# nktoan/h-edit

Hardware: AMD Instinct MI355X
Metric: edited images/sec (512^2, 50 steps, K Langevin) (higher is better)
Workload: dtype bf16

## Files before the change

h-edit_amd/csrc/store.h:

```cpp
#pragma once
#include <map>
#include <string>
#include <vector>

#include "../../include/hedit.h"
#include "common.h"

#pragma GCC visibility push(hidden)

enum class Pack {
  F32,
  Linear,
  Conv3,
  GegluRows,
  GegluBias,
  FfnLayer,
  FfnBias,
  ChainLayer,
  LinearT,
  Conv3Dgrad,
  Conv3S2Dgrad,
  FlipOIHW,
};

struct PackDst {
  Pack kind;
  void* dst;
  float scale = 1.f;
  long ld = 0;
  int which = 0, lay = 0;
};

struct ParamSlot {
  std::string name;
  size_t numel;
  int O, I;
  int ndim;
  int dims[4];
  bool loaded;
  PackDst to;
  std::vector<PackDst> more;
};

struct ParamStore {
  bool alloc_failed = false;
  bool finalized = false;
  std::vector<void*> owned;
  std::vector<ParamSlot> slots;
  std::map<std::string, int> index;
};

void* store_alloc(ParamStore* h, size_t bytes);
void store_free(ParamStore* h);
template <class T>
T* dalloc(ParamStore* h, size_t n) { return reinterpret_cast<T*>(store_alloc(h, n * sizeof(T))); }

ParamSlot& add_slot(ParamStore* h, const std::string& name, Pack kind, void* dst, size_t numel, int O, int I, int ndim,
                    int d0, int d1, int d2, int d3);
float* vec(ParamStore* h, const std::string& name, int n, float* dst = nullptr);
float* mat(ParamStore* h, const std::string& name, int O, int I);
float* f32conv(ParamStore* h, const std::string& name, int O, int I, int k);
bf16_t* lin(ParamStore* h, const std::string& name, int O, int I, bool conv1x1 = false, bf16_t* dst = nullptr, float scale = 1.f);
bf16_t* conv3(ParamStore* h, const std::string& name, int O, int I);
void* add_dst(ParamStore* h, Pack kind, void* dst, size_t bytes, float scale, long ld);
template <class T>
T* twin(ParamStore* h, Pack kind, size_t n, T* dst = nullptr, float scale = 1.f, long ld = 0) {
  return reinterpret_cast<T*>(add_dst(h, kind, dst, n * sizeof(T), scale, ld));
}

// ... 46 lines not shown
```

h-edit_amd/csrc/store.hip:

```cpp
#include "store.h"

#include "kernels.h"

#define TRY(expr)                        \
  do {                                   \
    int _rc = (expr);                    \
    if (_rc != HEDIT_OK) return _rc;     \
  } while (0)

void* store_alloc(ParamStore* h, size_t bytes) {
  void* p = nullptr;
  if (hipMalloc(&p, bytes > 0 ? bytes : 16) != hipSuccess) {
    h->alloc_failed = true;
    return nullptr;
  }
  h->owned.push_back(p);
  return p;
}

void store_free(ParamStore* h) {
  for (void* p : h->owned) if (p) (void)hipFree(p);
  h->owned.clear();
}

// ... 39 lines not shown

static int pack(const ParamSlot& s, const PackDst& d, const float* w, hipStream_t st) {
  bf16_t* d16 = reinterpret_cast<bf16_t*>(d.dst);
  float* d32 = reinterpret_cast<float*>(d.dst);
  switch (d.kind) {
    case Pack::F32: HIP_TRY(hipMemcpyAsync(d.dst, w, s.numel * sizeof(float), hipMemcpyDeviceToDevice, st)); return HEDIT_OK;
    case Pack::Linear: return pack_linear_launch(w, d16, (long)s.numel, d.scale, st);
    case Pack::Conv3: return pack_conv3x3_launch(w, d16, s.O, s.I, st);
    case Pack::GegluRows: return pack_geglu_rows_launch(w, d16, nullptr, s.O, s.I, st);
    case Pack::GegluBias: return pack_geglu_rows_launch(w, nullptr, d32, (int)s.numel, 1, st);
    case Pack::FfnLayer: return ffn_pack_launch(w, d.which, 1, 1, d16, st);
    case Pack::FfnBias: return ffn_pack_bias_launch(w, d32, st);
    case Pack::ChainLayer: return lin_chain_pack_launch(w, d.which, d.scale, d.lay, d16, st);
    case Pack::LinearT: return pack_linear_t_launch(w, d16, s.O, s.I, st, d.scale, d.ld);
    case Pack::Conv3Dgrad: return pack_conv3x3_dgrad_launch(w, d16, s.O, s.I, st);
    case Pack::Conv3S2Dgrad: return pack_conv3x3_s2_dgrad_launch(w, d16, s.O, s.I, st);
    case Pack::FlipOIHW: return flip_oihw_launch(w, d32, s.O, s.I, s.dims[2], st);
  }
  return HEDIT_ERR_STATE;
}

int store_load(ParamStore* h, const char* what, const char* name, const float* w, size_t numel, hipStream_t st) {
  h->finalized = false;
  auto it = h->index.find(name);
  if (it == h->index.end()) {
    hedit_set_error(std::string("unknown ") + what + (*what ? " " : "") + "parameter: " + name);
    return HEDIT_ERR_ARG;
  }
  ParamSlot& s = h->slots[it->second];
  if (s.numel != numel) {
    hedit_set_error(std::string("size mismatch for ") + name + ": expected " + std::to_string(s.numel) + ", got " + std::to_string(numel));
    return HEDIT_ERR_ARG;
  }
  TRY(pack(s, s.to, w, st));
  for (const PackDst& d : s.more) TRY(pack(s, d, w, st));
  s.loaded = true;
  return HEDIT_OK;
}

int store_missing(const ParamStore* h) {
  int m = 0;
  for (auto& s : h->slots) m += s.loaded ? 0 : 1;
  return m;
}
int store_num_params(const ParamStore* h) { return h ? (int)h->slots.size() : 0; }
const char* store_param_name(const ParamStore* h, int i) {
// ... 33 lines not shown
```

h-edit_amd/csrc/unet.hip:

```cpp
#include <array>
#include <map>
#include <string>
#include <vector>

#include "exec.h"
#include "kernels.h"
#include "store.h"

namespace {

struct Res {
  int cin, cout, temb_off;
  float *n1g, *n1b, *n2g, *n2b, *conv2_b, *sc_b;
  bf16_t *conv1, *conv2, *sc_w;
  bf16_t *conv1_t = nullptr, *conv2_t = nullptr, *sc_t = nullptr;
};

struct Attn {
  int C;
  float *gn_g, *gn_b, *pin_b, *ln1g, *ln1b, *ln2g, *ln2b, *ln3g, *ln3b, *o1_b, *o2_b, *ff1_b, *ff2_b, *pout_b;
  bf16_t *pin, *w_qk, *w_v1, *w_o1, *w_q2, *w_k2, *w_v2, *w_o2, *ff1, *ff2, *pout;
  bf16_t *frs = nullptr, *k1s = nullptr, *ffs = nullptr;
  float* ff1_bp = nullptr;
  int ctx_off = 0;
// ... 14 lines not shown

}

struct HEDIT_HANDLE hedit_unet : ParamStore {
  hedit_unet_cfg cfg;
  int temb_dim = 0, temb_total = 0;
  float *conv_in_w = nullptr, *conv_in_b = nullptr, *te1_b = nullptr, *te2_b = nullptr;
  bf16_t *te1_w = nullptr, *te2_w = nullptr, *temb_w_all = nullptr, *conv_out_w = nullptr;
  float *temb_b_all = nullptr, *conv1_b_all = nullptr, *gn_out_g = nullptr, *gn_out_b = nullptr, *conv_out_b = nullptr;
  std::vector<Block> down, up;
  Res mid_res[2];
  Attn mid_attn;
  int32_t* iota = nullptr;
  int iota_cap = 0;
  bool prof_on = false;
  std::vector<hipEvent_t> prof_pool;
  struct ProfRec { int kind; double flops, bytes; int e0, e1; int m = 0, n = 0, k = 0, tag = 0; };
  std::vector<ProfRec> prof_recs;
  size_t prof_next = 0;
  hedit_attn_hook_fn hook = nullptr;
  void* hook_user = nullptr;
  bf16_t *wk2_all = nullptr, *wv2_all = nullptr;
  int ctx_n = 0, ctx_next = 0;
  std::map<std::array<int, 4>, size_t> ws_cache;
  bool grad = false;
  bf16_t* conv_in_t = nullptr;
  float *conv_out_t = nullptr, *zero_bias = nullptr;
  void* tape = nullptr;
  void (*tape_free)(void*) = nullptr;
  bf16_t* wkv2_t = nullptr;
};

namespace {

void grad_lin(hedit_unet* h, int O, int I, float scale, bf16_t** t, bf16_t** fwd = nullptr) {
  if (!h->grad) return;
  *t = twin<bf16_t>(h, Pack::LinearT, (size_t)O * I, nullptr, scale);
  if (fwd) *fwd = twin<bf16_t>(h, Pack::Linear, (size_t)O * I, *fwd, scale);
}

Res make_res(hedit_unet* h, const std::string& pre, int cin, int cout, int& temb_off) {
  Res r{};
  r.cin = cin; r.cout = cout; r.temb_off = temb_off;
  r.n1g = vec(h, pre + ".norm1.weight", cin);
  r.n1b = vec(h, pre + ".norm1.bias", cin);
  r.conv1 = conv3(h, pre + ".conv1.weight", cout, cin);
// ... 495 lines not shown
}

int broadcast_stem(Fwd& f, size_t row_elems, bf16_t** x, bf16_t** t1, bf16_t** q2, int D) {
  bf16_t** narrow[3] = {x, t1, q2};
  bf16_t* wide[3];
  const void* src[3];
  void* dst[3];
  for (int i = 0; i < 3; ++i) {
    TRY(aalloc(f, &wide[i], (size_t)f.B * row_elems));
    src[i] = *narrow[i];
    dst[i] = wide[i];
  }
  {
    ProfScope ps(f, PK_OTHER, 0.0, 3.0 * (D + f.B) * (double)row_elems * sizeof(bf16_t));
    RUN(f, gather_rows_launch(src, dst, 3, f.B, (long)(row_elems * sizeof(bf16_t)), *f.map, f.st));
  }
  for (int i = 0; i < 3; ++i) {
    f.ar.free(*narrow[i]);
    *narrow[i] = wide[i];
  }
  return HEDIT_OK;
}

int forward_impl(hedit_unet* h, const float* x, float t, const float* ctx, int B, int H0, int W0,
                 const hedit_p2p_plan* plan, float* eps_out, void* ws, size_t ws_bytes, hipStream_t st,
                 bool dry, size_t* peak, int D = 0, const RowMap* map = nullptr) {
  const hedit_unet_cfg& c = h->cfg;
  Fwd f;
  f.h = h; f.B = B; f.st = st; f.plan = plan; f.map = map;
  f.ar.base = reinterpret_cast<char*>(ws); f.ar.cap = ws_bytes; f.ar.dry = dry;
  const int ch0 = c.block_out_channels[0];

  if (!dry && h->iota_cap < B) {
    hedit_set_error("batch larger than " + std::to_string(h->iota_cap) + " rows");
    return HEDIT_ERR_ARG;
  }

  bf16_t* ctxb;
  TRY(aalloc(f, &ctxb, (size_t)B * HEDIT_CTXP * c.cross_attention_dim));
  RUN(f, ctx_pad_launch(ctx, ctxb, B, c.cross_attention_dim, st));
  f.ctxb = ctxb;
  {
    const int MC = B * HEDIT_CTXP;
    bf16_t *k2a, *vt2a;
    TRY(aalloc(f, &k2a, (size_t)MC * h->ctx_n));
    TRY(aalloc(f, &vt2a, (size_t)MC * h->ctx_n));
    TRY(linear(f, ctxb, MC, c.cross_attention_dim, h->wk2_all, h->ctx_n, nullptr, nullptr, k2a, h->ctx_n));
    TRY(linear(f, h->wv2_all, h->ctx_n, c.cross_attention_dim, ctxb, MC, nullptr, nullptr, vt2a, MC, 2));
    f.k2_all = k2a;
    f.vt2_all = vt2a;
  }

  float *te0, *te1, *te2, *temb_all;
  TRY(aalloc(f, &te0, (size_t)ch0));
  TRY(aalloc(f, &te1, (size_t)h->temb_dim));
  TRY(aalloc(f, &te2, (size_t)h->temb_dim));
  TRY(aalloc(f, &temb_all, (size_t)h->temb_total));
  RUN(f, timestep_embed_launch(t, te0, ch0, st));
  RUN(f, gemv_launch(h->te1_w, te0, h->te1_b, nullptr, te1, h->temb_dim, ch0, 0, st));
  RUN(f, gemv_launch(h->te2_w, te1, h->te2_b, nullptr, te2, h->temb_dim, h->temb_dim, 1, st));
  RUN(f, gemv_launch(h->temb_w_all, te2, h->temb_b_all, h->conv1_b_all, temb_all, h->temb_total, h->temb_dim, 1, st));
  f.temb_all = temb_all;

  int H = H0, W = W0;
  const bool share = D > 0 && stem_shareable(h, plan, D, B, H0 * W0);
  float* xrows = nullptr;
  if (D > 0 && !share) {
    const size_t img = (size_t)c.in_channels * H * W;
    TRY(aalloc(f, &xrows, (size_t)B * img));
    const void* src[1] = {x};
    void* dst[1] = {xrows};
    ProfScope ps(f, PK_OTHER, 0.0, (double)(D + B) * img * sizeof(float));
    RUN(f, gather_rows_launch(src, dst, 1, B, (long)(img * sizeof(float)), *map, st));
// ... 123 lines not shown
      const size_t M = (size_t)B * H * W;
      TRY(aalloc(f, &prod, M * 4));
      GemmParams p{};
      p.mode = 1; p.Hin = H; p.Win = W; p.Cin = ch0; p.Hout = H; p.Wout = W;
      p.A = a; p.W = h->conv_out_w; p.M = (int)M; p.N = 4; p.K = 9 * ch0; p.lda = ch0; p.raw_f32 = prod; p.ldc = 4;
      TRY(run_gemm(f, p));
      RUN(f, rows_to_nchw_launch(prod, h->conv_out_b, eps_out, B, (long)H * W, 4, 4, st));
      f.ar.free(prod);
    }
    f.ar.free(a);
    f.ar.free(cur);
  }
  if (peak) *peak = f.ar.peak;
  return HEDIT_OK;
}

}

#include "unetgrad.h"

static void unet_pre_destroy(hedit_unet* h) {
  drop_tape(h);
  for (hipEvent_t e : h->prof_pool) (void)hipEventDestroy(e);
}
HEDIT_LIFECYCLE(unet, hedit_unet, "", unet_pre_destroy)

static int create_impl(const hedit_unet_cfg* cfg, hedit_unet** out, bool grad, bool ctx = false) {
  ARG_CHECK(cfg && out, "null");
  ARG_CHECK(cfg->n_levels >= 2 && cfg->n_levels <= HEDIT_MAX_LEVELS, "n_levels");
  ARG_CHECK(cfg->in_channels <= 8 && cfg->out_channels <= 4, "in/out channels");
  ARG_CHECK(cfg->cross_attention_dim % 64 == 0, "cross_attention_dim % 64");
  for (int i = 0; i < cfg->n_levels; ++i) {
    ARG_CHECK(cfg->block_out_channels[i] % 64 == 0, "block_out_channels % 64");
    ARG_CHECK(cfg->block_out_channels[i] % cfg->norm_num_groups == 0, "channels % groups");
    const int d = cfg->block_out_channels[i] / cfg->heads;
    ARG_CHECK(d == 32 || d == 40 || d == 64 || d == 80 || d == 160, "head dim must be one of 32,40,64,80,160");
  }
  TRY(gemm_prepare());
  if (grad) ARG_CHECK(cfg->in_channels <= 4, "the input-gradient pass needs in_channels <= 4");
  hedit_unet* h = new hedit_unet();
  h->cfg = *cfg;
  h->grad = grad;
  const int* ch = cfg->block_out_channels;
  const int L = cfg->layers_per_block, n = cfg->n_levels;
  h->temb_dim = ch[0] * 4;

// ... 116 lines not shown
  return create_impl(cfg, out, true, true);
} catch (...) { return hedit_abi_catch(); }

int hedit_unet_param_bf16_exact(const hedit_unet* h, int i) try {
  return store_param_bf16_exact(h, i);
} catch (...) { (void)hedit_abi_catch(); return 0; }

size_t hedit_unet_workspace_bytes(hedit_unet* h, int B, int height, int width) try {
  if (!h) return 0;
  const std::array<int, 4> key{B, height, width, h->hook ? 1 : 0};
  auto it = h->ws_cache.find(key);
  if (it != h->ws_cache.end()) return it->second;
  size_t need = 0;
  for (int D = 0; D <= (B <= HEDIT_ROWMAP_MAX ? B : 0); ++D) {
    size_t peak = 0;
    if (forward_impl(h, nullptr, 0.f, nullptr, B, height, width, nullptr, nullptr, nullptr, 0, nullptr, true, &peak, D) != HEDIT_OK) return 0;
    if (peak > need) need = peak;
  }
  need += 4096;
  h->ws_cache[key] = need;
  return need;
} catch (...) { (void)hedit_abi_catch(); return 0; }

static int forward_checks(hedit_unet* h, const float* x, const float* ctx, int B, int height, int width, const hedit_p2p_plan* plan,
                          float* eps_out, void* workspace) {
  ARG_CHECK(h && x && ctx && eps_out && workspace, "null");
  ARG_CHECK(B >= 1, "B");
  const int div = 1 << (h->cfg.n_levels - 1);
  ARG_CHECK(height % div == 0 && width % div == 0, "latent size must be divisible by 2^(levels-1)");
  const int lowest = (height / div) * (width / div);
  ARG_CHECK(lowest % 64 == 0, "lowest-resolution level must have a multiple of 64 tokens");
  TRY(store_require_loaded(h, "UNet"));
  ARG_CHECK(!(h->hook && plan && plan->mode > 0), "an attention hook excludes the in-kernel edits of a plan (pass plan = NULL)");
  if (plan && plan->mode > 0) {
    ARG_CHECK(plan->n_pairs >= 0 && plan->n_pairs + plan->n_single > 0, "plan rows");
    ARG_CHECK(plan->n_pairs == 0 || (plan->pair_src && plan->pair_tar && plan->mixT && plan->bvec), "plan tables");
  }
  return HEDIT_OK;
}

int hedit_unet_forward(hedit_unet* h, const float* x, float t, const float* ctx, int B, int height, int width,
                       const hedit_p2p_plan* plan, float* eps_out, void* workspace, size_t workspace_bytes,
                       void* stream) try {
  TRY(forward_checks(h, x, ctx, B, height, width, plan, eps_out, workspace));
  return forward_impl(h, x, t, ctx, B, height, width, plan, eps_out, workspace, workspace_bytes,
                      reinterpret_cast<hipStream_t>(stream), false, nullptr);
} catch (...) { return hedit_abi_catch(); }

int hedit_unet_forward_shared(hedit_unet* h, const float* x, int D, const int* row_latent, float t, const float* ctx, int B,
                              int height, int width, const hedit_p2p_plan* plan, float* eps_out, void* workspace,
                              size_t workspace_bytes, void* stream) try {
  TRY(forward_checks(h, x, ctx, B, height, width, plan, eps_out, workspace));
  ARG_CHECK(row_latent && D >= 1 && D <= 65535, "row map");
  if (B > HEDIT_ROWMAP_MAX) {
    hedit_set_error("batch larger than " + std::to_string(HEDIT_ROWMAP_MAX) + " rows (the row map of shared latents)");
    return HEDIT_ERR_ARG;
  }
  ARG_CHECK(reinterpret_cast<uintptr_t>(x) % 16 == 0, "x must be 16-byte aligned");
  RowMap map{};
  for (int r = 0; r < B; ++r) {
    ARG_CHECK(row_latent[r] >= 0 && row_latent[r] < D, "row_latent entries must lie in [0, D)");
    map.src[r] = (uint16_t)row_latent[r];
  }
  return forward_impl(h, x, t, ctx, B, height, width, plan, eps_out, workspace, workspace_bytes,
                      reinterpret_cast<hipStream_t>(stream), false, nullptr, D, &map);
} catch (...) { return hedit_abi_catch(); }

size_t hedit_unet_grad_workspace_bytes(hedit_unet* h, int B, int height, int width) try {
  if (!h || !h->grad || check_grad_shape(h, B, height, width) != HEDIT_OK) return 0;
  GradTape T;
  tape_init(T, h, B, height, width, nullptr, 0, nullptr, true);
  float dummy = 0.f;
  int rc = forward_keep_impl(h, T, nullptr, 0.f, nullptr, nullptr);
  if (rc == HEDIT_OK) rc = backward_impl(h, T, &dummy, &dummy);
  if (h->wkv2_t) {
    if (rc == HEDIT_OK) rc = backward_impl(h, T, &dummy, &dummy, &dummy);
    if (rc == HEDIT_OK) rc = backward_impl(h, T, &dummy, nullptr, &dummy);
  }
  return dry_run_bytes(rc, T.f.ar.peak);
} catch (...) { (void)hedit_abi_catch(); return 0; }

int hedit_unet_forward_keep(hedit_unet* h, const float* x, float t, const float* ctx, int B, int height, int width, float* eps,
                            void* workspace, size_t workspace_bytes, void* stream) try {
  ARG_CHECK(h && x && ctx && eps && workspace, "null");
  TRY(check_grad_shape(h, B, height, width));
  TRY(check_grad_handle(h, "hedit_unet_forward_keep"));
  drop_tape(h);
  GradTape* T = new GradTape();
// ... 172 lines not shown
```

h-edit_amd/hedit/_lib.py:

```python
import ctypes as C
import os

_HERE = os.path.dirname(os.path.abspath(__file__))
STORAGE = os.environ.get("HEDIT_STORAGE", "bf16").lower()
if STORAGE not in ("bf16", "f16"):
    raise ValueError(f"HEDIT_STORAGE must be bf16 or f16, not {STORAGE!r}")
LIB_PATH = os.path.join(_HERE, "libhedit_hip_f16.so" if STORAGE == "f16" else "libhedit_hip.so")
HEDIT_MAX_LEVELS = 8


class UnetCfg(C.Structure):
    _fields_ = [("in_channels", C.c_int), ("out_channels", C.c_int), ("sample_size", C.c_int),
                ("n_levels", C.c_int),
                ("block_out_channels", C.c_int * HEDIT_MAX_LEVELS),
                ("down_has_attn", C.c_int * HEDIT_MAX_LEVELS),
                ("up_has_attn", C.c_int * HEDIT_MAX_LEVELS),
                ("layers_per_block", C.c_int), ("cross_attention_dim", C.c_int),
                ("heads", C.c_int), ("norm_num_groups", C.c_int)]


class VaeCfg(C.Structure):
    _fields_ = [("in_channels", C.c_int), ("latent_channels", C.c_int), ("n_levels", C.c_int),
                ("block_out_channels", C.c_int * 4), ("layers_per_block", C.c_int),
                ("norm_num_groups", C.c_int)]
# ... 40 lines not shown
def _family(name, cfg, finalizes, workspace_args):
    sigs = {"create": (C.c_int, ([C.POINTER(cfg)] if cfg else []) + [C.POINTER(C.c_void_p)]),
            "destroy": (None, [C.c_void_p]),
            "num_params": (C.c_int, [C.c_void_p]),
            "param_name": (C.c_char_p, [C.c_void_p, C.c_int]),
            "param_shape": (C.c_int, [C.c_void_p, C.c_int, C.POINTER(C.c_int), C.POINTER(C.c_int)]),
            "load": (C.c_int, [C.c_void_p, C.c_char_p, C.c_void_p, C.c_size_t, C.c_void_p]),
            "missing": (C.c_int, [C.c_void_p]),
            "workspace_bytes": (C.c_size_t, [C.c_void_p] + workspace_args)}
    if finalizes:
        sigs["finalize"] = (C.c_int, [C.c_void_p, C.c_void_p])
    return {f"hedit_{name}_{k}": v for k, v in sigs.items()}


_SIGS = {    "hedit_last_error": (C.c_char_p, []),
    "hedit_version": (C.c_int, []),
    **_family("unet", UnetCfg, False, [C.c_int] * 3),
    "hedit_unet_param_bf16_exact": (C.c_int, [C.c_void_p, C.c_int]),
    "hedit_unet_forward": (C.c_int, [C.c_void_p, C.c_void_p, C.c_float, C.c_void_p, C.c_int, C.c_int,
                                     C.c_int, C.POINTER(P2PPlan), C.c_void_p, C.c_void_p, C.c_size_t,
                                     C.c_void_p]),
    "hedit_unet_forward_shared": (C.c_int, [C.c_void_p, C.c_void_p, C.c_int, C.POINTER(C.c_int), C.c_float, C.c_void_p, C.c_int,
                                            C.c_int, C.c_int, C.POINTER(P2PPlan), C.c_void_p, C.c_void_p, C.c_size_t, C.c_void_p]),
    "hedit_unet_create_grad": (C.c_int, [C.POINTER(UnetCfg), C.POINTER(C.c_void_p)]),
    "hedit_unet_grad_workspace_bytes": (C.c_size_t, [C.c_void_p, C.c_int, C.c_int, C.c_int]),
    "hedit_unet_forward_keep": (C.c_int, [C.c_void_p, C.c_void_p, C.c_float, C.c_void_p, C.c_int, C.c_int, C.c_int, C.c_void_p,
                                          C.c_void_p, C.c_size_t, C.c_void_p]),
    "hedit_unet_backward": (C.c_int, [C.c_void_p, C.c_void_p, C.c_void_p, C.c_void_p, C.c_void_p]),
    "hedit_unet_create_grad_ctx": (C.c_int, [C.POINTER(UnetCfg), C.POINTER(C.c_void_p)]),
    "hedit_unet_backward_ctx": (C.c_int, [C.c_void_p, C.c_void_p, C.c_void_p, C.c_void_p, C.c_void_p, C.c_void_p]),
    "hedit_unet_release": (None, [C.c_void_p]),
    "hedit_unet_vjp": (C.c_int, [C.c_void_p, C.c_void_p, C.c_float, C.c_void_p, C.c_void_p, C.c_int, C.c_int, C.c_int, C.c_void_p,
                                 C.c_void_p, C.c_void_p, C.c_size_t, C.c_void_p]),
    "hedit_unet_set_attn_hook": (C.c_int, [C.c_void_p, C.c_void_p, C.c_void_p]),
    "hedit_unet_num_store_layers": (C.c_int, [C.c_void_p, C.c_int, C.c_int]),
    "hedit_unet_store_layer_info": (C.c_int, [C.c_void_p, C.c_int, C.c_int, C.c_int, C.POINTER(C.c_int),
                                              C.POINTER(C.c_int)]),
    "hedit_prof_enable": (C.c_int, [C.c_void_p, C.c_int, C.c_int]),
    "hedit_prof_reset": (C.c_int, [C.c_void_p]),
    "hedit_prof_collect": (C.c_int, [C.c_void_p, C.c_int, C.POINTER(C.c_double), C.POINTER(C.c_double),
                                     C.POINTER(C.c_int64)]),
    "hedit_prof_collect_bytes": (C.c_int, [C.c_void_p, C.c_int, C.POINTER(C.c_double)]),
    "hedit_prof_records": (C.c_int, [C.c_void_p, C.POINTER(C.c_double), C.c_int, C.POINTER(C.c_int)]),
    "hedit_step_base": (C.c_int, [C.c_void_p, C.c_void_p, C.c_void_p, C.c_void_p, C.c_int, C.c_int,
                                  C.c_int, C.POINTER(StepCoef), C.c_void_p]),
    "hedit_step_pair": (C.c_int, [C.c_void_p, C.c_void_p, C.c_void_p, C.c_void_p, C.c_void_p, C.c_int, C.c_int, C.c_int,
# ... 205 lines not shown
```

h-edit_amd/hedit/engine.py:

```python
import ctypes as C

import torch

from . import _lib


def _f(x):
    return float(x)


class Schedule:

    def __init__(self, scheduler):
        self.s = scheduler
        self.ab = scheduler.alphas_cumprod.float().cpu()
        self.final = scheduler.final_alpha_cumprod.float().cpu() if isinstance(
            scheduler.final_alpha_cumprod, torch.Tensor) else torch.tensor(float(scheduler.final_alpha_cumprod))
        self.T = scheduler.num_inference_steps
        self.n_train = scheduler.config.num_train_timesteps

    def ab_prev(self, t):
        p = t - self.n_train // self.T
        return self.ab[p] if p >= 0 else self.final

# ... 131 lines not shown
            _lib.check(self.lib.hedit_step_ef_style(_lib.ptr(e_u), _lib.ptr(e_c), elems, _lib.ptr(dx), _lib.ptr(g_z),
                                                    _lib.ptr(x_prev_tar[lo:hi]), _lib.ptr(out[lo:hi]), m, elems, a, float(weight),
                                                    st()))
        return out

    def encode(self, prompts):
        if getattr(self.model.text_encoder, "batch_invariant", False):
            tok = self.model.tokenizer(list(prompts), padding="max_length", max_length=self.model.tokenizer.model_max_length,
                                       truncation=True, return_tensors="pt")
            with torch.no_grad():
                return self.model.text_encoder(tok.input_ids)[0].float()
        out = []
        for p in prompts:
            tok = self.model.tokenizer([p], padding="max_length", max_length=self.model.tokenizer.model_max_length,
                                       truncation=True, return_tensors="pt")
            with torch.no_grad():
                out.append(self.model.text_encoder(tok.input_ids.to(self.dev))[0].float())
        return torch.cat(out)

    @torch.no_grad()
    def run(self, xT, zs, prompt_pairs, cfg_scales, controller=None, eta=1.0, p2p=True, implicit=True,
            K=1, w_rec=0.1, after_skip_steps=None, ddim_inv=False, ctx=None, fuse_src_pass=False,
            reuse_orig_eps=False, style=None, rec_pull=True):
        if style is not None and not (p2p and implicit):
            raise ValueError("style guidance is defined for the implicit P2P loop only (n-style h_edit.py)")
        sch = self.model.scheduler
        S = Schedule(sch)
        T = sch.num_inference_steps
        if after_skip_steps is None:
            after_skip_steps = T
        n = xT.shape[0]
        dev = self.dev
        xT = xT.to(device=dev, dtype=torch.float32)
        if zs is not None:
            zs = zs.to(device=dev, dtype=torch.float32).contiguous()
        if ctx is None:
            null = self.encode([""])
            src = self.encode([p[0] for p in prompt_pairs])
            tar = self.encode([p[1] for p in prompt_pairs])
        else:
            null, src, tar = (c.to(device=dev, dtype=torch.float32) for c in ctx)
        nulln = null.expand(n, -1, -1) if null.shape[0] == 1 else null
        ctx_base4 = torch.cat([nulln, nulln, src, src]).contiguous()
        ctx_base2 = torch.cat([nulln, src]).contiguous()
        ctx_edit = torch.cat([nulln, nulln, src, tar]).contiguous()
        ctx_src = src.contiguous()
        ctx_edit5 = torch.cat([nulln, nulln, src, tar, src]).contiguous() if fuse_src_pass else None

        ts = [int(v) for v in sch.timesteps]
        op = ts[-after_skip_steps:]
        ahead = ts[-(after_skip_steps + 1)] if after_skip_steps != T else -1
        xt = torch.cat([xT, xT]).contiguous()
        x_prev = torch.empty_like(xt)
        off = None

        from .p2p.ptp_classes import runs_in_python
        foreign = runs_in_python(controller)
        if foreign:
            if n != 1 or fuse_src_pass or reuse_orig_eps:
                raise ValueError("a foreign controller runs one image at a time, without fuse_src_pass / reuse_orig_eps "
                                 "(it sees the reference's 4-row batch)")
            if not callable(controller):
                raise TypeError("a foreign controller must be callable as controller(attn, is_cross, place_in_unet, save_attn)")
        step_cb = getattr(controller, "step_callback", None) if controller is not None else None
        if step_cb is not None and not callable(step_cb):
            raise TypeError("controller.step_callback must be callable as step_callback(x_t) -> x_t")

        share = self.share_latents

        def unet_rows(parts, blocks, t, ctx_rows, plan=None):
            if not share:
                return self.unet.forward_raw(torch.cat([parts[b] for b in blocks]), t, ctx_rows, plan)
            lat = parts[0] if len(parts) == 1 else torch.cat(parts)
            return self.unet.forward_raw(lat, t, ctx_rows, plan, row_latent=[b * n + j for b in blocks for j in range(n)])

        def p2p_pass(parts, blocks, t, save):
            rows = len(blocks) * n
            if foreign:
                return self.unet.forward_hooked(torch.cat([parts[b] for b in blocks]), t, ctx_edit, controller, save)
            plan = controller._plan(self.unet, rows, xT.shape[2], xT.shape[3], save) if controller is not None else None
            e = unet_rows(parts, blocks, t, ctx_edit5 if rows == 5 * n else ctx_edit, plan)
            if controller is not None:
                controller._after_pass(save)
            return e

        carry = None
        reuse = reuse_orig_eps and p2p and implicit
        for i, t in enumerate(op):
            idx = T - i - (T - after_skip_steps + 1)
            z = zs[idx] if zs is not None else None
            tt = op[i + 1] if i < len(op) - 1 else 0
            eta_i = float(eta[idx]) if isinstance(eta, (list, tuple)) else float(eta)
            coef = S.step_coef(t, tt, eta_i, ddim_inv, cfg_scales, w_rec)

            if (not p2p) and implicit and i == 0 and ahead != -1:
                xe = xt[n:]
                e = unet_rows([xe], (0, 0, 0, 0), t, ctx_edit, off)
                c0 = S.step_coef(t, tt, eta_i, ddim_inv, cfg_scales, w_rec, coeff=S.edit_coeff(ahead, t, eta_i, ddim_inv))
                new = torch.empty_like(xe)
                self.step_update(e[0:n], e[2 * n:3 * n], e[n:2 * n], e[3 * n:], xe, xe, new, n, False, c0)
                xt = torch.cat([xt[:n], new]).contiguous()

# ... 315 lines not shown
```

h-edit_amd/hedit/unet.py:

```python
import ctypes as C
import hashlib
import math

import torch

from . import _lib
from .native import NativeOwner

SD15_CONFIG = dict(in_channels=4, out_channels=4, sample_size=64,
                   block_out_channels=(320, 640, 1280, 1280),
                   down_block_types=("CrossAttnDownBlock2D", "CrossAttnDownBlock2D",
                                     "CrossAttnDownBlock2D", "DownBlock2D"),
                   up_block_types=("UpBlock2D", "CrossAttnUpBlock2D", "CrossAttnUpBlock2D",
                                   "CrossAttnUpBlock2D"),
                   layers_per_block=2, cross_attention_dim=768, attention_head_dim=8,
                   norm_num_groups=32)

TINY_CONFIG = dict(in_channels=4, out_channels=4, sample_size=32,
                   block_out_channels=(64, 128, 128),
                   down_block_types=("CrossAttnDownBlock2D", "CrossAttnDownBlock2D", "DownBlock2D"),
                   up_block_types=("UpBlock2D", "CrossAttnUpBlock2D", "CrossAttnUpBlock2D"),
                   layers_per_block=2, cross_attention_dim=64, attention_head_dim=2,
                   norm_num_groups=32)

# ... 33 lines not shown
    def forward(ctx, sample, enc, model, t):
        ctx.model = model
        ctx.ticket, eps = model._keep(sample.detach(), t, enc)
        ctx.shape = sample.shape
        ctx.enc_shape = enc.shape
        return eps

    @staticmethod
    def backward(ctx, g):
        m = ctx.model
        if m._ticket != ctx.ticket:
            raise RuntimeError("hedit.UNet2DConditionModel: the kept forward of this graph was dropped by a later model call")
        g = g.detach().to(dtype=torch.float32).contiguous()
        want_x, want_c = ctx.needs_input_grad[0], ctx.needs_input_grad[1]
        dx = torch.empty(ctx.shape, dtype=torch.float32, device=m.device) if want_x else None
        dc = torch.empty(ctx.enc_shape, dtype=torch.float32, device=m.device) if want_c else None
        with torch.cuda.device(m.device):
            if want_c:
                _lib.check(m._lib.hedit_unet_backward_ctx(m._h, _lib.ptr(g), _lib.ptr(dx) if want_x else None, _lib.ptr(dc),
                                                          _lib.ptr(m._gws), _lib.cur_stream()))
            elif want_x:
                _lib.check(m._lib.hedit_unet_backward(m._h, _lib.ptr(g), _lib.ptr(dx), _lib.ptr(m._gws), _lib.cur_stream()))
        return dx, dc, None, None


class UNet2DConditionModel(NativeOwner):
    _family, _finalizes = "unet", False
    _tickets = 0

    def __init__(self, config=None, device="cuda:0", grad=False):
        cfg = dict(SD15_CONFIG)
        cfg.update(config or {})
        self.config = cfg
        self.device = torch.device(device)
        if self.device.type != "cuda":
            raise RuntimeError("hedit.UNet2DConditionModel runs on the GPU only (HIP kernels)")
        self.in_channels = cfg["in_channels"]
        self.sample_size = cfg["sample_size"]
        c = _lib.UnetCfg()
        c.in_channels, c.out_channels, c.sample_size = cfg["in_channels"], cfg["out_channels"], cfg["sample_size"]
        ch = list(cfg["block_out_channels"])
        c.n_levels = len(ch)
        for i, v in enumerate(ch):
            c.block_out_channels[i] = v
            c.down_has_attn[i] = int(cfg["down_block_types"][i].startswith("CrossAttn"))
            c.up_has_attn[i] = int(cfg["up_block_types"][i].startswith("CrossAttn"))
        c.layers_per_block = cfg["layers_per_block"]
        c.cross_attention_dim = cfg["cross_attention_dim"]
        c.heads = cfg["attention_head_dim"]
        c.norm_num_groups = cfg["norm_num_groups"]
        self._cfg_struct = c
        if isinstance(grad, str) and grad != "context":
            raise ValueError(f'grad must be False, True or "context", got {grad!r}')
        self._native_build(self.device, None, c, create="create_grad_ctx" if grad == "context" else "create_grad" if grad else "create")
        self.grad = bool(grad)
        self.grad_context = grad == "context"
        self._ticket = 0
        self._gws = None
        self.param_shapes = self._native_param_shapes()
        self.bf16_exact = {name for i, name in enumerate(self.param_shapes) if self._lib.hedit_unet_param_bf16_exact(self._h, i)}
        self._procs = {n: AttnProcessor() for n in self._processor_names()}
        self.heads = cfg["attention_head_dim"]

    load_state_dict = NativeOwner._native_load

    def init_random(self, seed=0):
        sd = random_state_dict(self.param_shapes, seed)
        self.load_state_dict(sd)
        return sd

    def zero_grad(self, *a, **k):
        return None

    def _processor_names(self):
        cfg = self.config
        names = []
        L = cfg["layers_per_block"]
# ... 73 lines not shown
            out[k] = (ms.value, fl.value, n.value)
        return out

    def prof_collect_bytes(self):
        out = {}
        b = C.c_double()
        for i, k in enumerate(self.PROF_KINDS):
            _lib.check(self._lib.hedit_prof_collect_bytes(self._h, i, C.byref(b)))
            out[k] = b.value
        return out

    def prof_records(self, max_rows=16384):
        import numpy as np
        torch.cuda.synchronize(self.device)
        rows = np.zeros((max_rows, 8), dtype=np.float64)
        n = C.c_int()
        _lib.check(self._lib.hedit_prof_records(self._h, rows.ctypes.data_as(C.POINTER(C.c_double)), max_rows, C.byref(n)))
        return rows[:n.value]

    def forward_raw(self, sample, t, ctx, plan=None, out=None, row_latent=None):
        B, Cc, H, W = sample.shape
        if row_latent is not None:
            B = len(row_latent)
        if sample.dtype != torch.float32 or ctx.dtype != torch.float32:
            raise TypeError("sample and encoder_hidden_states must be float32")
        if ctx.shape != (B, 77, self.config["cross_attention_dim"]):
            raise ValueError(f"encoder_hidden_states must be ({B}, 77, {self.config['cross_attention_dim']}), "
                             f"got {tuple(ctx.shape)}")
        sample = sample.contiguous()
        ctx = ctx.contiguous()
        if out is None:
            out = torch.empty(B, self.config["out_channels"], H, W, dtype=torch.float32, device=sample.device)
        ws = self._workspace(B, H, W)
        if row_latent is None:
            _lib.check(self._lib.hedit_unet_forward(
                self._h, _lib.ptr(sample), C.c_float(float(t)), _lib.ptr(ctx), B, H, W,
                C.byref(plan) if plan is not None else None, _lib.ptr(out), _lib.ptr(ws), ws.numel(),
                _lib.cur_stream()))
            return out
        if sample.data_ptr() % 16:
            sample = sample.clone()
        _lib.check(self._lib.hedit_unet_forward_shared(
            self._h, _lib.ptr(sample), sample.shape[0], (C.c_int * B)(*row_latent), C.c_float(float(t)), _lib.ptr(ctx), B, H, W,
            C.byref(plan) if plan is not None else None, _lib.ptr(out), _lib.ptr(ws), ws.numel(),
            _lib.cur_stream()))
        return out

    def _release(self):
        if self._ticket:
            self._lib.hedit_unet_release(self._h)
            self._ticket = 0

    def _keep(self, sample, t, ctx):
        sample, ctx = sample.contiguous(), ctx.detach().contiguous()
        B, _, H, W = sample.shape
        if ctx.shape != (B, 77, self.config["cross_attention_dim"]):
            raise ValueError(f"encoder_hidden_states must be ({B}, 77, {self.config['cross_attention_dim']}), got {tuple(ctx.shape)}")
        need = self._lib.hedit_unet_grad_workspace_bytes(self._h, B, H, W)
        if need == 0:
            raise _lib.HipError("gradient workspace planning failed: " + self._lib.hedit_last_error().decode())
        self._grow("_gws", need, self.device)
        eps = torch.empty(B, self.config["out_channels"], H, W, dtype=torch.float32, device=self.device)
        with torch.cuda.device(self.device):
            _lib.check(self._lib.hedit_unet_forward_keep(self._h, _lib.ptr(sample), C.c_float(float(t)), _lib.ptr(ctx), B, H, W,
                                                         _lib.ptr(eps), _lib.ptr(self._gws), self._gws.numel(), _lib.cur_stream()))
        UNet2DConditionModel._tickets += 1
        self._ticket = UNet2DConditionModel._tickets
        return self._ticket, eps
# ... 78 lines not shown
```

include/hedit.h:

```cpp
#ifndef HEDIT_H
#define HEDIT_H
#include <stddef.h>
#include <stdint.h>

#ifdef __cplusplus
extern "C" {
#endif

#define HEDIT_MAX_LEVELS 8

typedef struct hedit_unet hedit_unet;

typedef struct {
  int in_channels, out_channels, sample_size;
  int n_levels;
  int block_out_channels[HEDIT_MAX_LEVELS];
  int down_has_attn[HEDIT_MAX_LEVELS];
  int up_has_attn[HEDIT_MAX_LEVELS];
  int layers_per_block;
  int cross_attention_dim;
  int heads;
  int norm_num_groups;
} hedit_unet_cfg;

// ... 21 lines not shown
typedef struct {
  float sqrt_ab_t, sqrt_1m_ab_t, sqrt_ab_prev, dir_coef, noise_coef;
  float w_src, w_hat, w_tar, coeff, w_rec;
} hedit_step_coef;

const char* hedit_last_error(void);
int hedit_version(void);

int hedit_unet_create(const hedit_unet_cfg* cfg, hedit_unet** out);
void hedit_unet_destroy(hedit_unet* h);
int hedit_unet_num_params(const hedit_unet* h);
const char* hedit_unet_param_name(const hedit_unet* h, int i);
int hedit_unet_param_shape(const hedit_unet* h, int i, int* ndim, int* dims4);
int hedit_unet_load(hedit_unet* h, const char* name, const float* w, size_t numel, void* stream);
int hedit_unet_param_bf16_exact(const hedit_unet* h, int i);
int hedit_unet_missing(const hedit_unet* h);
size_t hedit_unet_workspace_bytes(hedit_unet* h, int B, int height, int width);
int hedit_unet_forward(hedit_unet* h, const float* x, float t, const float* ctx, int B, int height,
                       int width, const hedit_p2p_plan* plan, float* eps_out, void* workspace,
                       size_t workspace_bytes, void* stream);
int hedit_unet_forward_shared(hedit_unet* h, const float* x, int D, const int* row_latent, float t, const float* ctx, int B,
                              int height, int width, const hedit_p2p_plan* plan, float* eps_out, void* workspace,
                              size_t workspace_bytes, void* stream);
typedef int (*hedit_attn_hook_fn)(void* user, float* probs, int batch_heads, int n_query, int n_key, int is_cross, int place,
                                  int layer, void* stream);
int hedit_unet_set_attn_hook(hedit_unet* h, hedit_attn_hook_fn fn, void* user);
int hedit_unet_num_store_layers(const hedit_unet* h, int height, int width);
int hedit_unet_store_layer_info(const hedit_unet* h, int height, int width, int i, int* tokens,
                                int* place );

int hedit_unet_create_grad(const hedit_unet_cfg* cfg, hedit_unet** out);
int hedit_unet_create_grad_ctx(const hedit_unet_cfg* cfg, hedit_unet** out);
int hedit_unet_backward_ctx(hedit_unet* h, const float* d_eps, float* d_x, float* d_ctx, void* workspace, void* stream);
size_t hedit_unet_grad_workspace_bytes(hedit_unet* h, int B, int height, int width);
int hedit_unet_forward_keep(hedit_unet* h, const float* x, float t, const float* ctx, int B, int height, int width, float* eps,
                            void* workspace, size_t workspace_bytes, void* stream);
int hedit_unet_backward(hedit_unet* h, const float* d_eps, float* d_x, void* workspace, void* stream);
void hedit_unet_release(hedit_unet* h);
int hedit_unet_vjp(hedit_unet* h, const float* x, float t, const float* ctx, const float* d_eps, int B, int height, int width,
                   float* d_x, float* eps, void* workspace, size_t workspace_bytes, void* stream);

int hedit_prof_enable(hedit_unet* h, int on, int max_records);
int hedit_prof_reset(hedit_unet* h);
int hedit_prof_collect(hedit_unet* h, int kind, double* total_ms, double* total_flops, int64_t* count);
int hedit_prof_collect_bytes(hedit_unet* h, int kind, double* total_bytes);
int hedit_prof_records(hedit_unet* h, double* rows, int max_rows, int* n_rows);
// ... 312 lines not shown
```

Baseline: 2.660.

## Bind text contexts once and reuse cross-attention K/V projections across steps

Adds a context-binding API that pads the text context and projects all cross-attention keys and values once, storing them in persistent device buffers. The edit engine binds each prompt context at the start of a run and passes bound handles to the UNet, so every denoising step and Langevin iteration skips the context pad and two projection GEMMs. Bindings are checked against a parameter-load counter and released after the run, at the cost of extra device memory and per-run bind and sync overhead.

```diff
diff --git a/h-edit_amd/csrc/store.h b/h-edit_amd/csrc/store.h
--- a/h-edit_amd/csrc/store.h
+++ b/h-edit_amd/csrc/store.h
@@ -45,6 +45,7 @@
 struct ParamStore {
   bool alloc_failed = false;
   bool finalized = false;
+  unsigned loads = 0;
   std::vector<void*> owned;
   std::vector<ParamSlot> slots;
   std::map<std::string, int> index;
diff --git a/h-edit_amd/csrc/store.hip b/h-edit_amd/csrc/store.hip
--- a/h-edit_amd/csrc/store.hip
+++ b/h-edit_amd/csrc/store.hip
@@ -85,6 +85,7 @@
 
 int store_load(ParamStore* h, const char* what, const char* name, const float* w, size_t numel, hipStream_t st) {
   h->finalized = false;
+  ++h->loads;
   auto it = h->index.find(name);
   if (it == h->index.end()) {
     hedit_set_error(std::string("unknown ") + what + (*what ? " " : "") + "parameter: " + name);
diff --git a/h-edit_amd/csrc/unet.hip b/h-edit_amd/csrc/unet.hip
--- a/h-edit_amd/csrc/unet.hip
+++ b/h-edit_amd/csrc/unet.hip
@@ -60,6 +60,9 @@
   void* hook_user = nullptr;
   bf16_t *wk2_all = nullptr, *wv2_all = nullptr;
   int ctx_n = 0, ctx_next = 0;
+  struct BoundCtx { int B = 0; unsigned loads = 0; bf16_t *k2 = nullptr, *vt2 = nullptr; };
+  std::map<int, BoundCtx> bound;
+  int bound_next = 1;
   std::map<std::array<int, 4>, size_t> ws_cache;
   bool grad = false;
   bf16_t* conv_in_t = nullptr;
@@ -601,9 +604,21 @@
   return HEDIT_OK;
 }
 
+int project_context(Fwd& f, const float* ctx, bf16_t* ctxb, bf16_t* k2a, bf16_t* vt2a) {
+  const hedit_unet* h = f.h;
+  const int dim = h->cfg.cross_attention_dim, MC = f.B * HEDIT_CTXP;
+  RUN(f, ctx_pad_launch(ctx, ctxb, f.B, dim, f.st));
+  TRY(linear(f, ctxb, MC, dim, h->wk2_all, h->ctx_n, nullptr, nullptr, k2a, h->ctx_n));
+  TRY(linear(f, h->wv2_all, h->ctx_n, dim, ctxb, MC, nullptr, nullptr, vt2a, MC, 2));
+  f.ctxb = ctxb;
+  f.k2_all = k2a;
+  f.vt2_all = vt2a;
+  return HEDIT_OK;
+}
+
 int forward_impl(hedit_unet* h, const float* x, float t, const float* ctx, int B, int H0, int W0,
                  const hedit_p2p_plan* plan, float* eps_out, void* ws, size_t ws_bytes, hipStream_t st,
-                 bool dry, size_t* peak, int D = 0, const RowMap* map = nullptr) {
+                 bool dry, size_t* peak, int D = 0, const RowMap* map = nullptr, const hedit_unet::BoundCtx* bound = nullptr) {
   const hedit_unet_cfg& c = h->cfg;
   Fwd f;
   f.h = h; f.B = B; f.st = st; f.plan = plan; f.map = map;
@@ -615,19 +630,17 @@
     return HEDIT_ERR_ARG;
   }
 
-  bf16_t* ctxb;
-  TRY(aalloc(f, &ctxb, (size_t)B * HEDIT_CTXP * c.cross_attention_dim));
-  RUN(f, ctx_pad_launch(ctx, ctxb, B, c.cross_attention_dim, st));
-  f.ctxb = ctxb;
-  {
-    const int MC = B * HEDIT_CTXP;
-    bf16_t *k2a, *vt2a;
-    TRY(aalloc(f, &k2a, (size_t)MC * h->ctx_n));
-    TRY(aalloc(f, &vt2a, (size_t)MC * h->ctx_n));
-    TRY(linear(f, ctxb, MC, c.cross_attention_dim, h->wk2_all, h->ctx_n, nullptr, nullptr, k2a, h->ctx_n));
-    TRY(linear(f, h->wv2_all, h->ctx_n, c.cross_attention_dim, ctxb, MC, nullptr, nullptr, vt2a, MC, 2));
-    f.k2_all = k2a;
-    f.vt2_all = vt2a;
+  if (bound) {
+    f.ctxb = nullptr;
+    f.k2_all = bound->k2;
+    f.vt2_all = bound->vt2;
+  } else {
+    const size_t MC = (size_t)B * HEDIT_CTXP;
+    bf16_t *ctxb, *k2a, *vt2a;
+    TRY(aalloc(f, &ctxb, MC * c.cross_attention_dim));
+    TRY(aalloc(f, &k2a, MC * h->ctx_n));
+    TRY(aalloc(f, &vt2a, MC * h->ctx_n));
+    TRY(project_context(f, ctx, ctxb, k2a, vt2a));
   }
 
   float *te0, *te1, *te2, *temb_all;
@@ -797,6 +810,11 @@
 static void unet_pre_destroy(hedit_unet* h) {
   drop_tape(h);
   for (hipEvent_t e : h->prof_pool) (void)hipEventDestroy(e);
+  for (auto& kv : h->bound) {
+    (void)hipFree(kv.second.k2);
+    (void)hipFree(kv.second.vt2);
+  }
+  h->bound.clear();
 }
 HEDIT_LIFECYCLE(unet, hedit_unet, "", unet_pre_destroy)
 
@@ -959,7 +977,7 @@
   return need;
 } catch (...) { (void)hedit_abi_catch(); return 0; }
 
-static int forward_checks(hedit_unet* h, const float* x, const float* ctx, int B, int height, int width, const hedit_p2p_plan* plan,
+static int forward_checks(hedit_unet* h, const float* x, const void* ctx, int B, int height, int width, const hedit_p2p_plan* plan,
                           float* eps_out, void* workspace) {
   ARG_CHECK(h && x && ctx && eps_out && workspace, "null");
   ARG_CHECK(B >= 1, "B");
@@ -984,10 +1002,29 @@
                       reinterpret_cast<hipStream_t>(stream), false, nullptr);
 } catch (...) { return hedit_abi_catch(); }
 
-int hedit_unet_forward_shared(hedit_unet* h, const float* x, int D, const int* row_latent, float t, const float* ctx, int B,
-                              int height, int width, const hedit_p2p_plan* plan, float* eps_out, void* workspace,
-                              size_t workspace_bytes, void* stream) try {
-  TRY(forward_checks(h, x, ctx, B, height, width, plan, eps_out, workspace));
+static int bound_lookup(hedit_unet* h, int id, int B, const hedit_unet::BoundCtx** out) {
+  ARG_CHECK(h, "null");
+  auto it = h->bound.find(id);
+  if (it == h->bound.end()) {
+    hedit_set_error("no bound context with id " + std::to_string(id) + " on this handle (hedit_unet_context_bind)");
+    return HEDIT_ERR_ARG;
+  }
+  if (it->second.B != B) {
+    hedit_set_error("the context was bound with " + std::to_string(it->second.B) + " rows, the call has " + std::to_string(B));
+    return HEDIT_ERR_ARG;
+  }
+  if (it->second.loads != h->loads) {
+    hedit_set_error("parameters were loaded after the context was bound: release it and bind again");
+    return HEDIT_ERR_STATE;
+  }
+  *out = &it->second;
+  return HEDIT_OK;
+}
+
+static int forward_shared_checked(hedit_unet* h, const float* x, int D, const int* row_latent, float t, const float* ctx,
+                                  const hedit_unet::BoundCtx* bound, int B, int height, int width, const hedit_p2p_plan* plan,
+                                  float* eps_out, void* workspace, size_t workspace_bytes, void* stream) {
+  TRY(forward_checks(h, x, bound ? (const void*)bound : (const void*)ctx, B, height, width, plan, eps_out, workspace));
   ARG_CHECK(row_latent && D >= 1 && D <= 65535, "row map");
   if (B > HEDIT_ROWMAP_MAX) {
     hedit_set_error("batch larger than " + std::to_string(HEDIT_ROWMAP_MAX) + " rows (the row map of shared latents)");
@@ -1000,7 +1037,91 @@
     map.src[r] = (uint16_t)row_latent[r];
   }
   return forward_impl(h, x, t, ctx, B, height, width, plan, eps_out, workspace, workspace_bytes,
-                      reinterpret_cast<hipStream_t>(stream), false, nullptr, D, &map);
+                      reinterpret_cast<hipStream_t>(stream), false, nullptr, D, &map, bound);
+}
+
+int hedit_unet_forward_shared(hedit_unet* h, const float* x, int D, const int* row_latent, float t, const float* ctx, int B,
+                              int height, int width, const hedit_p2p_plan* plan, float* eps_out, void* workspace,
+                              size_t workspace_bytes, void* stream) try {
+  return forward_shared_checked(h, x, D, row_latent, t, ctx, nullptr, B, height, width, plan, eps_out, workspace, workspace_bytes, stream);
+} catch (...) { return hedit_abi_catch(); }
+
+int hedit_unet_context_bind(hedit_unet* h, const float* ctx, int B, void* stream, int* id) try {
+  ARG_CHECK(h && ctx && id, "null");
+  ARG_CHECK(B >= 1 && B <= h->iota_cap, "B");
+  TRY(store_require_loaded(h, "UNet"));
+  hipStream_t st = reinterpret_cast<hipStream_t>(stream);
+  const size_t MC = (size_t)B * HEDIT_CTXP, dim = h->cfg.cross_attention_dim;
+  Fwd f;
+  f.h = h; f.B = B; f.st = st; f.plan = nullptr;
+  f.ar.dry = true;
+  bf16_t* ctxb;
+  TRY(aalloc(f, &ctxb, MC * dim));
+  TRY(project_context(f, nullptr, ctxb, nullptr, nullptr));
+  const size_t scratch_bytes = f.ar.peak;
+  hedit_unet::BoundCtx bc;
+  bc.B = B; bc.loads = h->loads;
+  void* scratch = nullptr;
+  int rc = HEDIT_OK;
+  if (hipMalloc(&scratch, scratch_bytes) != hipSuccess || hipMalloc(reinterpret_cast<void**>(&bc.k2), MC * h->ctx_n * sizeof(bf16_t)) != hipSuccess ||
+      hipMalloc(reinterpret_cast<void**>(&bc.vt2), MC * h->ctx_n * sizeof(bf16_t)) != hipSuccess) {
+    (void)hipGetLastError();
+    hedit_set_error("hedit_unet_context_bind: out of device memory");
+    rc = HEDIT_ERR_HIP;
+  }
+  if (rc == HEDIT_OK) {
+    f.ar = Arena();
+    f.ar.base = reinterpret_cast<char*>(scratch); f.ar.cap = scratch_bytes;
+    rc = aalloc(f, &ctxb, MC * dim);
+    const bool prof = h->prof_on;
+    h->prof_on = false;
+    if (rc == HEDIT_OK) rc = project_context(f, ctx, ctxb, bc.k2, bc.vt2);
+    h->prof_on = prof;
+    if (hipStreamSynchronize(st) != hipSuccess && rc == HEDIT_OK) {
+      hedit_set_error("hedit_unet_context_bind: the projection launches failed");
+      rc = HEDIT_ERR_HIP;
+    }
+  }
+  if (scratch) (void)hipFree(scratch);
+  if (rc != HEDIT_OK) {
+    if (bc.k2) (void)hipFree(bc.k2);
+    if (bc.vt2) (void)hipFree(bc.vt2);
+    return rc;
+  }
+  *id = h->bound_next++;
+  h->bound[*id] = bc;
+  return HEDIT_OK;
+} catch (...) { return hedit_abi_catch(); }
+
+int hedit_unet_context_release(hedit_unet* h, int id) try {
+  ARG_CHECK(h, "null");
+  auto it = h->bound.find(id);
+  if (it == h->bound.end()) {
+    hedit_set_error("no bound context with id " + std::to_string(id) + " on this handle");
+    return HEDIT_ERR_ARG;
+  }
+  (void)hipFree(it->second.k2);
+  (void)hipFree(it->second.vt2);
+  h->bound.erase(it);
+  return HEDIT_OK;
+} catch (...) { return hedit_abi_catch(); }
+
+int hedit_unet_forward_bound(hedit_unet* h, const float* x, float t, int ctx_id, int B, int height, int width,
+                             const hedit_p2p_plan* plan, float* eps_out, void* workspace, size_t workspace_bytes,
+                             void* stream) try {
+  const hedit_unet::BoundCtx* bc = nullptr;
+  TRY(bound_lookup(h, ctx_id, B, &bc));
+  TRY(forward_checks(h, x, bc, B, height, width, plan, eps_out, workspace));
+  return forward_impl(h, x, t, nullptr, B, height, width, plan, eps_out, workspace, workspace_bytes,
+                      reinterpret_cast<hipStream_t>(stream), false, nullptr, 0, nullptr, bc);
+} catch (...) { return hedit_abi_catch(); }
+
+int hedit_unet_forward_shared_bound(hedit_unet* h, const float* x, int D, const int* row_latent, float t, int ctx_id, int B,
+                                    int height, int width, const hedit_p2p_plan* plan, float* eps_out, void* workspace,
+                                    size_t workspace_bytes, void* stream) try {
+  const hedit_unet::BoundCtx* bc = nullptr;
+  TRY(bound_lookup(h, ctx_id, B, &bc));
+  return forward_shared_checked(h, x, D, row_latent, t, nullptr, bc, B, height, width, plan, eps_out, workspace, workspace_bytes, stream);
 } catch (...) { return hedit_abi_catch(); }
 
 size_t hedit_unet_grad_workspace_bytes(hedit_unet* h, int B, int height, int width) try {
diff --git a/h-edit_amd/hedit/_lib.py b/h-edit_amd/hedit/_lib.py
--- a/h-edit_amd/hedit/_lib.py
+++ b/h-edit_amd/hedit/_lib.py
@@ -86,6 +86,14 @@
                                      C.c_void_p]),
     "hedit_unet_forward_shared": (C.c_int, [C.c_void_p, C.c_void_p, C.c_int, C.POINTER(C.c_int), C.c_float, C.c_void_p, C.c_int,
                                             C.c_int, C.c_int, C.POINTER(P2PPlan), C.c_void_p, C.c_void_p, C.c_size_t, C.c_void_p]),
+    "hedit_unet_context_bind": (C.c_int, [C.c_void_p, C.c_void_p, C.c_int, C.c_void_p, C.POINTER(C.c_int)]),
+    "hedit_unet_context_release": (C.c_int, [C.c_void_p, C.c_int]),
+    "hedit_unet_forward_bound": (C.c_int, [C.c_void_p, C.c_void_p, C.c_float, C.c_int, C.c_int, C.c_int,
+                                           C.c_int, C.POINTER(P2PPlan), C.c_void_p, C.c_void_p, C.c_size_t,
+                                           C.c_void_p]),
+    "hedit_unet_forward_shared_bound": (C.c_int, [C.c_void_p, C.c_void_p, C.c_int, C.POINTER(C.c_int), C.c_float, C.c_int, C.c_int,
+                                                  C.c_int, C.c_int, C.POINTER(P2PPlan), C.c_void_p, C.c_void_p, C.c_size_t,
+                                                  C.c_void_p]),
     "hedit_unet_create_grad": (C.c_int, [C.POINTER(UnetCfg), C.POINTER(C.c_void_p)]),
     "hedit_unet_grad_workspace_bytes": (C.c_size_t, [C.c_void_p, C.c_int, C.c_int, C.c_int]),
     "hedit_unet_forward_keep": (C.c_int, [C.c_void_p, C.c_void_p, C.c_float, C.c_void_p, C.c_int, C.c_int, C.c_int, C.c_void_p,
diff --git a/h-edit_amd/hedit/engine.py b/h-edit_amd/hedit/engine.py
--- a/h-edit_amd/hedit/engine.py
+++ b/h-edit_amd/hedit/engine.py
@@ -177,6 +177,16 @@
     def run(self, xT, zs, prompt_pairs, cfg_scales, controller=None, eta=1.0, p2p=True, implicit=True,
             K=1, w_rec=0.1, after_skip_steps=None, ddim_inv=False, ctx=None, fuse_src_pass=False,
             reuse_orig_eps=False, style=None, rec_pull=True):
+        held = []
+        try:
+            return self._run(held, xT, zs, prompt_pairs, cfg_scales, controller, eta, p2p, implicit, K, w_rec, after_skip_steps,
+                             ddim_inv, ctx, fuse_src_pass, reuse_orig_eps, style, rec_pull)
+        finally:
+            for b in held:
+                self.unet.release_context(b)
+
+    def _run(self, held, xT, zs, prompt_pairs, cfg_scales, controller, eta, p2p, implicit, K, w_rec, after_skip_steps, ddim_inv,
+             ctx, fuse_src_pass, reuse_orig_eps, style, rec_pull):
         if style is not None and not (p2p and implicit):
             raise ValueError("style guidance is defined for the implicit P2P loop only (n-style h_edit.py)")
         sch = self.model.scheduler
@@ -201,6 +211,20 @@
         ctx_edit = torch.cat([nulln, nulln, src, tar]).contiguous()
         ctx_src = src.contiguous()
         ctx_edit5 = torch.cat([nulln, nulln, src, tar, src]).contiguous() if fuse_src_pass else None
+        ctx_edit_rows = ctx_edit
+
+        def bind(c, used):
+            if not used or c is None:
+                return c
+            held.append(self.unet.bind_context(c))
+            return held[-1]
+
+        fused = p2p and implicit and fuse_src_pass
+        ctx_base4 = bind(ctx_base4, p2p)
+        ctx_base2 = bind(ctx_base2, not p2p or reuse_orig_eps)
+        ctx_edit = bind(ctx_edit, not fused)
+        ctx_src = bind(ctx_src, p2p and not fused)
+        ctx_edit5 = bind(ctx_edit5, fused)
 
         ts = [int(v) for v in sch.timesteps]
         op = ts[-after_skip_steps:]
@@ -232,7 +256,7 @@
         def p2p_pass(parts, blocks, t, save):
             rows = len(blocks) * n
             if foreign:
-                return self.unet.forward_hooked(torch.cat([parts[b] for b in blocks]), t, ctx_edit, controller, save)
+                return self.unet.forward_hooked(torch.cat([parts[b] for b in blocks]), t, ctx_edit_rows, controller, save)
             plan = controller._plan(self.unet, rows, xT.shape[2], xT.shape[3], save) if controller is not None else None
             e = unet_rows(parts, blocks, t, ctx_edit5 if rows == 5 * n else ctx_edit, plan)
             if controller is not None:
diff --git a/h-edit_amd/hedit/unet.py b/h-edit_amd/hedit/unet.py
--- a/h-edit_amd/hedit/unet.py
+++ b/h-edit_amd/hedit/unet.py
@@ -79,6 +79,13 @@
             elif want_x:
                 _lib.check(m._lib.hedit_unet_backward(m._h, _lib.ptr(g), _lib.ptr(dx), _lib.ptr(m._gws), _lib.cur_stream()))
         return dx, dc, None, None
+
+
+class BoundContext:
+    __slots__ = ("id", "rows", "handle")
+
+    def __init__(self, id, rows, handle):
+        self.id, self.rows, self.handle = id, rows, handle
 
 
 class UNet2DConditionModel(NativeOwner):
@@ -110,6 +117,7 @@
         if isinstance(grad, str) and grad != "context":
             raise ValueError(f'grad must be False, True or "context", got {grad!r}')
         self._native_build(self.device, None, c, create="create_grad_ctx" if grad == "context" else "create_grad" if grad else "create")
+        self._bound = {}
         self.grad = bool(grad)
         self.grad_context = grad == "context"
         self._ticket = 0
@@ -229,6 +237,8 @@
         B, Cc, H, W = sample.shape
         if row_latent is not None:
             B = len(row_latent)
+        if isinstance(ctx, BoundContext):
+            return self._forward_bound(sample, t, ctx, plan, out, row_latent, B)
         if sample.dtype != torch.float32 or ctx.dtype != torch.float32:
             raise TypeError("sample and encoder_hidden_states must be float32")
         if ctx.shape != (B, 77, self.config["cross_attention_dim"]):
@@ -251,6 +261,45 @@
             self._h, _lib.ptr(sample), sample.shape[0], (C.c_int * B)(*row_latent), C.c_float(float(t)), _lib.ptr(ctx), B, H, W,
             C.byref(plan) if plan is not None else None, _lib.ptr(out), _lib.ptr(ws), ws.numel(),
             _lib.cur_stream()))
+        return out
+
+    def bind_context(self, ctx):
+        if ctx.dtype != torch.float32 or ctx.dim() != 3 or ctx.shape[1:] != (77, self.config["cross_attention_dim"]):
+            raise ValueError(f"a context to bind must be float32 (B, 77, {self.config['cross_attention_dim']}), got "
+                             f"{ctx.dtype} {tuple(ctx.shape)}")
+        ctx = ctx.to(self.device).contiguous()
+        cid = C.c_int()
+        with torch.cuda.device(self.device):
+            _lib.check(self._lib.hedit_unet_context_bind(self._h, _lib.ptr(ctx), ctx.shape[0], _lib.cur_stream(), C.byref(cid)))
+        bound = BoundContext(cid.value, ctx.shape[0], self._h)
+        self._bound[bound.id] = bound
+        return bound
+
+    def release_context(self, bound):
+        if self._bound.pop(bound.id, None) is bound and bound.handle is self._h and self._h is not None:
+            _lib.check(self._lib.hedit_unet_context_release(self._h, bound.id))
+
+    def _forward_bound(self, sample, t, bound, plan, out, row_latent, B):
+        if self._bound.get(bound.id) is not bound or bound.handle is not self._h:
+            raise ValueError("this context is not bound on this model (released, or bound on another one)")
+        if sample.dtype != torch.float32:
+            raise TypeError("sample must be float32")
+        _, _, H, W = sample.shape
+        sample = sample.contiguous()
+        if out is None:
+            out = torch.empty(B, self.config["out_channels"], H, W, dtype=torch.float32, device=sample.device)
+        ws = self._workspace(B, H, W)
+        pl = C.byref(plan) if plan is not None else None
+        if row_latent is None:
+            _lib.check(self._lib.hedit_unet_forward_bound(
+                self._h, _lib.ptr(sample), C.c_float(float(t)), bound.id, B, H, W, pl, _lib.ptr(out), _lib.ptr(ws), ws.numel(),
+                _lib.cur_stream()))
+            return out
+        if sample.data_ptr() % 16:
+            sample = sample.clone()
+        _lib.check(self._lib.hedit_unet_forward_shared_bound(
+            self._h, _lib.ptr(sample), sample.shape[0], (C.c_int * B)(*row_latent), C.c_float(float(t)), bound.id, B, H, W,
+            pl, _lib.ptr(out), _lib.ptr(ws), ws.numel(), _lib.cur_stream()))
         return out
 
     def _release(self):
diff --git a/include/hedit.h b/include/hedit.h
--- a/include/hedit.h
+++ b/include/hedit.h
@@ -67,6 +67,14 @@
 int hedit_unet_forward_shared(hedit_unet* h, const float* x, int D, const int* row_latent, float t, const float* ctx, int B,
                               int height, int width, const hedit_p2p_plan* plan, float* eps_out, void* workspace,
                               size_t workspace_bytes, void* stream);
+int hedit_unet_context_bind(hedit_unet* h, const float* ctx, int B, void* stream, int* id);
+int hedit_unet_context_release(hedit_unet* h, int id);
+int hedit_unet_forward_bound(hedit_unet* h, const float* x, float t, int ctx_id, int B, int height, int width,
+                             const hedit_p2p_plan* plan, float* eps_out, void* workspace, size_t workspace_bytes,
+                             void* stream);
+int hedit_unet_forward_shared_bound(hedit_unet* h, const float* x, int D, const int* row_latent, float t, int ctx_id, int B,
+                                    int height, int width, const hedit_p2p_plan* plan, float* eps_out, void* workspace,
+                                    size_t workspace_bytes, void* stream);
 typedef int (*hedit_attn_hook_fn)(void* user, float* probs, int batch_heads, int n_query, int n_key, int is_cross, int place,
                                   int layer, void* stream);
 int hedit_unet_set_attn_hook(hedit_unet* h, hedit_attn_hook_fn fn, void* user);
```

Measured after the change: 2.672, median of 6. About the same (+0.4%).
